# dfki-asr/morphablegraphs

Hardware: AMD Instinct MI355X
Metric: motion-primitive samples scored+back-projected/sec; fraction of HBM roofline (higher is better)
Workload: dtype f32; 1 GPU; walk primitive L=40 F=156 D=79 NB=31 GMM k=8, batch=8192 candidates/GPU (BASELINE.json configs[1]); candidates_per_gpu=8192, global_candidates=8192, collective=none, clock_ramp_steps=1500

## Files before the change

include/mg_hip.h:

```cpp
#ifndef MG_HIP_H
#define MG_HIP_H

#include <stdint.h>

#ifdef __cplusplus
extern "C" {
#endif

typedef struct mg_context mg_context;
typedef struct mg_primitive mg_primitive;
typedef struct mg_time_grid mg_time_grid;
typedef struct mg_constraint_set mg_constraint_set;

enum {
    MG_OK = 0,
    MG_ERR_INVALID_ARGUMENT = -1,
    MG_ERR_NO_DEVICE = -2,
    MG_ERR_HIP = -3,
    MG_ERR_UNSUPPORTED = -4,
    MG_ERR_NOT_POSITIVE_DEFINITE = -5,
    MG_ERR_OUT_OF_MEMORY = -6
};

enum { MG_F32 = 0, MG_F64 = 1 };

enum {
    MG_PATH_AUTO = 0,
    MG_PATH_MFMA = 1,
    MG_PATH_DIRECT = 2
};

typedef struct mg_primitive_desc {
    int32_t n_basis;
    int32_t n_dim;
    int32_t n_components;
    int32_t n_canonical_frames;
    int32_t n_gmm;
    int32_t eigen_is_transposed;
    const double *eigen_vectors;
    const double *mean_vector;
    const double *translation_maxima;
    const double *knots;
    const double *gmm_weights;
    const double *gmm_means;
    const double *gmm_covars;
    int32_t n_gmm_dims;
    int32_t n_time_components;
    int32_t n_basis_time;
    int32_t reserved;
    const double *eigen_vectors_time;
    const double *mean_time_vector;
    const double *knots_time;
} mg_primitive_desc;

enum { MG_CONSTRAINT_POSITION = 0, MG_CONSTRAINT_DIRECTION_2D = 1, MG_CONSTRAINT_JOINT_POSITION = 2,
       MG_CONSTRAINT_JOINT_MIDPOINT = 3, MG_CONSTRAINT_JOINT_ORIENTATION = 4, MG_CONSTRAINT_LOOK_AT = 5,
       MG_CONSTRAINT_POSE = 6 ,
       MG_CONSTRAINT_VALUE_POSITION = 7, MG_CONSTRAINT_VALUE_HEADING = 8 };
#define MG_MAX_CHAIN 32
typedef struct mg_keyframe_constraint {
    int32_t type;
    int32_t joint;
    double canonical_keyframe;
    double weight_factor;
    double target[3];
    double ref_dir[3];
    int32_t joint2;
    int32_t reserved;
} mg_keyframe_constraint;

typedef struct mg_pose_constraint {
    int32_t n_points;
    int32_t has_velocity;
    const int32_t *joints;
    const double *points;
    const double *weights;
    double velocity[3];
} mg_pose_constraint;
#define MG_MAX_POSE_POINTS 64

typedef struct mg_skeleton_desc {
    int32_t n_joints;
    int32_t reserved;
    const int32_t *parents;
    const double *offsets;
    const int32_t *quat_channel;
} mg_skeleton_desc;

#define MG_ALIGN_START_POSE (-1)
typedef struct mg_alignment_desc {
    int32_t joint;
    int32_t reserved;
    double position[3];
    double heading[2];
    double ref_dir[3];
} mg_alignment_desc;

const char *mg_version(void);
const char *mg_last_error(void);
const char *mg_status_string(int status);

int mg_context_create(int device, void *stream, mg_context **out);
void mg_context_destroy(mg_context *ctx);
int mg_context_set_stream(mg_context *ctx, void *stream);
int mg_context_set_reserved_cus(mg_context *ctx, int32_t n);
#define MG_OPT_FORCE_VALU_SCORE 0
#define MG_OPT_FORCE_VALU_SAMPLE 1
#define MG_OPT_RING_SLOTS 2
#define MG_OPT_CHUNK_WINDOW 3
#define MG_OPT_CHUNK_SAMPLES 4
#define MG_OPT_FRAMES_KERNEL 5
#define MG_OPT_PLACED_FAST_PCT 6
#define MG_OPT_OPTIONS_STEP 7
#define MG_OPT_PLAIN_MALLOC 8
#define MG_OPT_GMM_KERNEL 9
#define MG_OPT_SCORE_KERNEL 10
#define MG_OPT_ROOT_MODE 11
#define MG_OPT_PLACED_HOLD 12
#define MG_OPT_TRAJECTORY_LANES 13
#define MG_OPT_TRAJECTORY_SEARCH 14
#define MG_OPT_COUNT 15
int mg_context_set_option(mg_context *ctx, int32_t option, int32_t value);
int mg_context_arena_begin(mg_context *ctx, int64_t block_bytes);
int mg_context_arena_end(mg_context *ctx);
int mg_context_arena_bytes(mg_context *ctx, int64_t *reserved, int64_t *used);
int mg_context_synchronize(mg_context *ctx);
int mg_context_device_info(mg_context *ctx, char *name, int32_t *n_cu, int64_t *total_mem);

int mg_device_malloc(mg_context *ctx, int64_t bytes, void **out_dev);
int mg_device_free(mg_context *ctx, void *ptr_dev);
int mg_context_trim_outputs(mg_context *ctx);
int mg_context_output_bytes(mg_context *ctx, int64_t *reserved, int64_t *in_use, int32_t *n_regions, int32_t *n_fast);
int mg_device_malloc_chunked(mg_context *ctx, int64_t bytes, int64_t chunk_bytes, void **out_dev);
int mg_device_malloc_placed(mg_context *ctx, int64_t bytes, int32_t max_candidates, void **out_dev, double *info4);
int mg_device_probe_placement(mg_context *ctx, void *buf_dev, int64_t bytes, double *info4);
int mg_device_placement_info(mg_context *ctx, const void *buf_dev, double *info4, double *tbps);
int mg_memcpy_h2d(mg_context *ctx, void *dst_dev, const void *src, int64_t bytes);
int mg_memcpy_d2h(mg_context *ctx, void *dst, const void *src_dev, int64_t bytes);
int mg_memset(mg_context *ctx, void *dst_dev, int value, int64_t bytes);

int mg_profile_enable(mg_context *ctx, int enabled);
int mg_profile_reset(mg_context *ctx);
int mg_profile_get(mg_context *ctx, int slot, double *total_ms, int64_t *launches);
int mg_profile_get_samples(mg_context *ctx, int slot, float *out_ms, int64_t capacity, int64_t *n);

#define MG_DIST_ID_BYTES 128
int mg_dist_unique_id(void *id_out);
int mg_dist_init(mg_context *ctx, int32_t rank, int32_t n_ranks, const void *id);
int mg_dist_all_gather(mg_context *ctx, const void *local_dev, void *gathered_dev, int64_t count, int dtype);
int mg_dist_broadcast(mg_context *ctx, void *buf_dev, int64_t bytes, int32_t root);
int mg_dist_finalize(mg_context *ctx);
int mg_dist_preflight(mg_context *ctx);
int mg_dist_info(mg_context *ctx, int32_t *out3);

int mg_primitive_create(mg_context *ctx, const mg_primitive_desc *desc, mg_primitive **out);
void mg_primitive_destroy(mg_primitive *prim);
int mg_primitive_info(const mg_primitive *prim, int32_t *out8);
int mg_primitive_info2(const mg_primitive *prim, int32_t *out4);
int mg_primitive_root_mode(const mg_primitive *prim, int32_t *split, double *estimate);
int mg_primitive_get_precisions_cholesky(const mg_primitive *prim, double *out);

int mg_time_function_canonical(mg_primitive *prim, const void *gamma_dev, int gamma_dtype, int64_t n_samples, int64_t ld,
                               double *out_dev);
int mg_time_function_canonical_host(mg_primitive *prim, const void *gamma, int gamma_dtype, int64_t n_samples, int64_t ld,
                                    double *out);
int mg_time_function_sample(mg_primitive *prim, const void *gamma, int dtype, int64_t n, int64_t ld, double speed, double *times, int32_t *lengths,
                            int32_t t_cap, double *canonical_out);
int mg_time_function_sample_rows(mg_primitive *prim, const void *gamma, int dtype, int64_t n, int64_t ld, double speed, double *times, int32_t *lengths,
                                 int32_t t_cap, int64_t row_pitch, double *canonical_out);
int mg_back_project_frames_at(mg_primitive *prim, const void *latents, int dtype, int64_t n, int64_t ld, const double *times, const int32_t *lengths,
                              int32_t t_cap, void *out, int out_dtype);

int mg_time_grid_create(mg_primitive *prim, const double *times, int32_t n_times, mg_time_grid **out);
void mg_time_grid_destroy(mg_time_grid *grid);
mg_time_grid *mg_primitive_canonical_grid(mg_primitive *prim);
int mg_time_grid_size(const mg_time_grid *grid);
int mg_time_grid_get_tables(const mg_time_grid *grid, int32_t *i0, double *weights, double *times);

int mg_joint_positions(mg_context *ctx, const mg_skeleton_desc *skeleton, const int32_t *joints, int32_t n_out,
                       const double *frames_dev, int64_t n_frames, int32_t n_dim, double *out_dev);

typedef struct mg_trajectory mg_trajectory;
int mg_trajectory_create(mg_primitive *prim, const double *control_points, int32_t n_points, int32_t granularity, mg_trajectory **out);
void mg_trajectory_destroy(mg_trajectory *trajectory);
int mg_score_trajectory(mg_primitive *prim, const mg_trajectory *trajectory, const mg_time_grid *grid, const void *latents_dev,
                        int latent_dtype, int64_t n_samples, int64_t ld, double min_u, double weight, const mg_alignment_desc *alignment,
                        double *errors_dev, int accumulate, double *residuals_dev);
int mg_score_trajectories(int32_t n, mg_primitive *const *prims, const mg_trajectory *const *trajectories, const void *const *latents_dev,
                          int latent_dtype, int64_t n_samples, const int64_t *ld, const double *min_u, const double *weight,
                          const mg_alignment_desc *const *alignments, double *const *errors_dev, int accumulate);

int mg_score_trajectory_points(mg_primitive *prim, const mg_trajectory *trajectory, const double *points_dev, int64_t n_samples, int32_t n_times,
                               double min_u, double weight, double *errors_dev, int accumulate, double *residuals_dev);

int mg_trajectory_closest_points(mg_primitive *prim, const mg_trajectory *trajectory, const double *points_dev, int64_t n_samples, int32_t n_times,
                                 double min_u, double *params_dev, double *distances_dev, int32_t *evaluations_dev);

#define MG_FRAME_CA_POSITION 1
#define MG_FRAME_DISCRETE_TRAJECTORY 2
#define MG_FRAME_LOCAL_TRAJECTORY 3
#define MG_FRAME_TRAJECTORY_SET 4
#define MG_FRAME_JOINT_ROTATION 5
#define MG_FRAME_JOINT_TRAJECTORY 6
#define MG_FRAME_MAX_JOINTS 8
typedef struct mg_frame_constraint_desc {
    int32_t type;
    int32_t n_frames;
    int32_t n_points;
    int32_t n_joints;
    double weight;
    double target[3];
    int32_t axis_on[3];
    int32_t quat_channel;
    const double *points_dev;
    double start_arc;
    const mg_trajectory *trajectories[MG_FRAME_MAX_JOINTS];
    double arc0[MG_FRAME_MAX_JOINTS], range_start[MG_FRAME_MAX_JOINTS], range_end[MG_FRAME_MAX_JOINTS];
    int32_t has_range[MG_FRAME_MAX_JOINTS];
    double quaternion[4];
} mg_frame_constraint_desc;
int mg_align_frames(mg_primitive *prim, double *frames_dev, int64_t n_samples, int32_t n_times, const double *vals_dev, int32_t n_vals,
                    const mg_alignment_desc *alignment);
int mg_frame_constraint_width(const mg_frame_constraint_desc *constraint, int32_t n_times);
int mg_score_frame_constraint(mg_primitive *prim, const mg_frame_constraint_desc *constraint, const double *tracks_dev, int64_t n_samples,
                              int32_t n_times, int32_t n_joints, double *errors_dev, int accumulate, double *residuals_dev);
typedef struct mg_track_plan mg_track_plan;
int mg_track_plan_create(mg_primitive *prim, const mg_skeleton_desc *skeleton, int32_t n_requests, const int32_t *n_joints, const int32_t *joints,
                         int32_t align_joint, mg_track_plan **out);
void mg_track_plan_destroy(mg_track_plan *plan);
int mg_joint_tracks(mg_track_plan *plan, const void *latents, int dtype, int64_t n_samples, int64_t ld, const mg_alignment_desc *alignment,
                    const mg_time_grid *const *grids, double *const *tracks_dev);
int mg_score_frame_constraints(mg_primitive *prim, int32_t n_constraints, const mg_frame_constraint_desc *const *constraints, const double *const *tracks_dev,
                               const int32_t *n_times, const int32_t *n_joints, int64_t n_samples, double *errors_dev, int accumulate,
                               double *const *residuals_dev);

#define MG_TRACK_MAX_REQUESTS 4
#define MG_FRAME_LIST_MAX 4
int mg_options_frame_lists(int32_t n_options, mg_primitive *const *prims, mg_track_plan *const *plans, const void *const *latents_dev, int latent_dtype,
                           int64_t n_samples, const int64_t *ld, const mg_alignment_desc *const *alignments, const mg_time_grid *const *grids,
                           double *const *tracks_dev, const int32_t *n_constraints, const mg_frame_constraint_desc *const *constraints,
                           const int32_t *request_of, double *const *errors_dev, void *results_dev, int64_t result_stride, void *results_host);


int mg_back_project_frames(mg_primitive *prim, const mg_time_grid *grid,
                           const void *latents_dev, int latent_dtype, int64_t n_samples, int64_t ld,
                           float *frames_dev, int path);

int mg_back_project_frames_f64(mg_primitive *prim, const mg_time_grid *grid,
                               const void *latents_dev, int latent_dtype, int64_t n_samples, int64_t ld,
                               double *frames_dev);

int mg_back_project_coeffs(mg_primitive *prim, const void *latents_dev, int latent_dtype,
                           int64_t n_samples, int64_t ld, void *coeffs_dev, int out_dtype);

int mg_spline_evaluate(mg_primitive *prim, const mg_time_grid *grid, const double *coeffs_dev,
                       int64_t n_splines, double *frames_dev);

int mg_gmm_log_prob(mg_primitive *prim, const void *x_dev, int x_dtype, int64_t n_samples, int64_t ld,
                    void *logp_dev, int out_dtype);

int mg_gmm_log_prob_jac(mg_primitive *prim, const void *x_dev, int x_dtype, int64_t n_samples, int64_t ld,
                        double *jac_dev);

int mg_gmm_sample(mg_primitive *prim, int64_t n_samples, const int64_t *counts, uint64_t seed,
                  void *x_dev, int x_dtype, int64_t ld, int32_t *component_dev);
int mg_gmm_sample_rows(mg_primitive *prim, int64_t n_samples, const int64_t *counts, uint64_t seed, int64_t row_begin, int64_t row_count,
                       void *x_dev, int x_dtype, int64_t ld, int32_t *component_dev);

int mg_constraint_set_create(mg_primitive *prim, const mg_keyframe_constraint *cons, int32_t n,
                             mg_constraint_set **out);
int mg_constraint_set_create_fk(mg_primitive *prim, const mg_skeleton_desc *skeleton,
                                const mg_keyframe_constraint *cons, int32_t n, mg_constraint_set **out);
int mg_constraint_set_create_aligned(mg_primitive *prim, const mg_skeleton_desc *skeleton,
                                     const mg_keyframe_constraint *cons, int32_t n,
// ... 166 lines not shown
```

morphablegraphs_amd/_capi.py:

```python
import ctypes as C
import functools
import itertools
import os

import numpy as np

HERE = os.path.dirname(os.path.abspath(__file__))
LIB_PATH = os.path.join(HERE, "csrc", "libmg_hip.so")

MG_OK = 0
MG_ERR_INVALID_ARGUMENT = -1
MG_ERR_UNSUPPORTED = -4
MG_F32, MG_F64 = 0, 1
MG_PATH_AUTO, MG_PATH_MFMA, MG_PATH_DIRECT = 0, 1, 2
MG_ALIGN_START_POSE = -1
MG_OPT_FORCE_VALU_SCORE, MG_OPT_FORCE_VALU_SAMPLE, MG_OPT_RING_SLOTS, MG_OPT_CHUNK_WINDOW, MG_OPT_CHUNK_SAMPLES = 0, 1, 2, 3, 4
MG_OPT_FRAMES_KERNEL = 5
MG_OPT_PLACED_FAST_PCT = 6
MG_OPT_OPTIONS_STEP = 7
MG_OPT_PLAIN_MALLOC = 8
MG_OPT_GMM_KERNEL = 9
MG_OPT_SCORE_KERNEL = 10
MG_OPT_ROOT_MODE = 11
MG_OPT_PLACED_HOLD = 12
MG_OPT_TRAJECTORY_LANES = 13
MG_OPT_TRAJECTORY_SEARCH = 14
MG_OPT_COUNT = 15
MG_CONSTRAINT_POSITION, MG_CONSTRAINT_DIRECTION_2D, MG_CONSTRAINT_JOINT_POSITION = 0, 1, 2
MG_CONSTRAINT_JOINT_MIDPOINT, MG_CONSTRAINT_JOINT_ORIENTATION, MG_CONSTRAINT_LOOK_AT, MG_CONSTRAINT_POSE = 3, 4, 5, 6
MG_CONSTRAINT_VALUE_POSITION, MG_CONSTRAINT_VALUE_HEADING = 7, 8
PROFILE_SLOTS = {"frames": 0, "gmm_log_prob": 1, "score_constraints": 2, "argmin": 3,
                 "gmm_sample": 4, "spline_evaluate": 5, "step": 6, "options_step": 7, "joint_tracks": 8, "frame_constraints": 9, "trajectory": 10,
                 "cluster_tree_search": 11, "walk_frames": 12}
MG_TREE_MAX_DEPTH, MG_TREE_MAX_CHILDREN, MG_TREE_MAX_CANDIDATES = 64, 256, 64
MG_TREE_TIE, MG_TREE_NO_RESULT, MG_TREE_OVERFLOW, MG_TREE_NO_MEAN = 1, 2, 4, 8
MG_KD_MAX_DEPTH = 64
TREE_SEARCH_RECORD = np.dtype([("row", "<i8"), ("leaf", "<i4"), ("flags", "<i4"), ("evaluations", "<i8"), ("value", "<f8")])
MG_WALK_MAX_STEPS = 64
MG_WALK_TILE = 32
MG_FUSED_MAX_OPTIONS = 24


@functools.lru_cache(maxsize=None)
def _option_record(stride):
    return np.dtype([("index", "<i8"), ("error", "<f8"), ("latent", "<f8", ((stride - 16) // 8,))])


def option_records(raw, m, stride):
    return raw[:m * stride].copy().view(_option_record(stride))


EXPORTED_SYMBOLS = [
    "mg_version", "mg_last_error", "mg_status_string",
    "mg_context_create", "mg_context_destroy", "mg_context_set_stream", "mg_context_set_reserved_cus", "mg_context_set_option", "mg_context_arena_begin", "mg_context_arena_end", "mg_context_arena_bytes", "mg_context_synchronize",
    "mg_dist_unique_id", "mg_dist_init", "mg_dist_all_gather", "mg_dist_finalize", "mg_dist_preflight", "mg_dist_info",
    "mg_context_device_info", "mg_device_malloc", "mg_device_malloc_chunked", "mg_device_malloc_placed", "mg_device_probe_placement", "mg_device_placement_info", "mg_device_free", "mg_context_trim_outputs", "mg_context_output_bytes", "mg_memcpy_h2d", "mg_memcpy_d2h",
    "mg_memset", "mg_profile_enable", "mg_profile_reset", "mg_profile_get", "mg_profile_get_samples",
    "mg_primitive_create", "mg_primitive_destroy", "mg_primitive_info", "mg_primitive_info2", "mg_primitive_root_mode", "mg_primitive_get_precisions_cholesky",
    "mg_time_function_canonical", "mg_time_function_canonical_host", "mg_time_function_sample", "mg_time_function_sample_rows", "mg_back_project_frames_at",
    "mg_trajectory_create", "mg_trajectory_destroy", "mg_score_trajectory", "mg_score_trajectories", "mg_score_trajectory_points", "mg_trajectory_closest_points", "mg_joint_positions",
    "mg_time_grid_create", "mg_time_grid_destroy", "mg_primitive_canonical_grid", "mg_time_grid_size",
    "mg_time_grid_get_tables",
    "mg_back_project_frames", "mg_back_project_frames_f64", "mg_back_project_coeffs", "mg_spline_evaluate",
    "mg_gmm_log_prob", "mg_gmm_sample", "mg_constraint_set_create", "mg_constraint_set_destroy",
    "mg_score_constraints", "mg_argmin_first", "mg_argmin_first_dev", "mg_step_frames_and_logp", "mg_step_plan", "mg_step_plan_for", "mg_step_plan_dtype",
    "mg_back_project_frames_host", "mg_back_project_frames_f64_host", "mg_back_project_coeffs_host",
    "mg_spline_evaluate_host", "mg_gmm_log_prob_host", "mg_gmm_sample_host", "mg_score_constraints_host",
    "mg_score_constraint_residuals", "mg_objective_error_and_naturalness", "mg_gmm_log_prob_jac", "mg_score_constraint_residuals_host",
    "mg_gmm_log_prob_jac_host", "mg_constraint_set_create_fk", "mg_constraint_set_create_aligned", "mg_constraint_set_create_full", "mg_constraint_set_update", "mg_best_candidate", "mg_best_candidate_host",
    "mg_align_frames", "mg_frame_constraint_width", "mg_score_frame_constraint", "mg_score_frame_constraints", "mg_options_frame_lists", "mg_track_plan_create", "mg_track_plan_destroy", "mg_joint_tracks",
    "mg_score_constraint_residuals_chained", "mg_option_step", "mg_options_step", "mg_options_step_device_counts", "mg_option_step_rows", "mg_options_step_rows", "mg_gmm_sample_rows", "mg_dist_broadcast",
    "mg_cluster_tree_create", "mg_cluster_tree_destroy", "mg_cluster_tree_search", "mg_cluster_tree_search_host",
    "mg_cluster_tree_create_kd", "mg_kmeans_segments", "mg_gmm_em_fit",
    "mg_spline_fit_batch", "mg_pca_fit", "mg_pca_project", "mg_pca_backproject",
    "mg_dtw_distance_grids", "mg_dtw_paths", "mg_warp_motions", "mg_dtw_pair_costs",
    "mg_keyframe_distances", "mg_segment_search",
    "mg_align_motions_spatially", "mg_prepare_aligned_frames",
    "mg_walk_frames", "mg_walk_frames_host",
]


class MGError(RuntimeError):
    def __init__(self, status, message):
        RuntimeError.__init__(self, "libmg_hip status %d: %s" % (status, message))
        self.status = status


class PrimitiveDesc(C.Structure):
    _fields_ = [("n_basis", C.c_int32), ("n_dim", C.c_int32), ("n_components", C.c_int32),
                ("n_canonical_frames", C.c_int32), ("n_gmm", C.c_int32), ("eigen_is_transposed", C.c_int32),
                ("eigen_vectors", C.c_void_p), ("mean_vector", C.c_void_p), ("translation_maxima", C.c_void_p),
                ("knots", C.c_void_p), ("gmm_weights", C.c_void_p), ("gmm_means", C.c_void_p),
                ("gmm_covars", C.c_void_p), ("n_gmm_dims", C.c_int32), ("n_time_components", C.c_int32),
                ("n_basis_time", C.c_int32), ("reserved", C.c_int32), ("eigen_vectors_time", C.c_void_p),
                ("mean_time_vector", C.c_void_p), ("knots_time", C.c_void_p)]


class KeyframeConstraint(C.Structure):
    _fields_ = [("type", C.c_int32), ("joint", C.c_int32), ("canonical_keyframe", C.c_double),
                ("weight_factor", C.c_double), ("target", C.c_double * 3), ("ref_dir", C.c_double * 3),
                ("joint2", C.c_int32), ("reserved", C.c_int32)]


class PoseConstraintDesc(C.Structure):
    _fields_ = [("n_points", C.c_int32), ("has_velocity", C.c_int32), ("joints", C.c_void_p), ("points", C.c_void_p),
                ("weights", C.c_void_p), ("velocity", C.c_double * 3)]


class SkeletonDesc(C.Structure):
    _fields_ = [("n_joints", C.c_int32), ("reserved", C.c_int32), ("parents", C.c_void_p), ("offsets", C.c_void_p),
                ("quat_channel", C.c_void_p)]


class AlignmentDesc(C.Structure):
    _fields_ = [("joint", C.c_int32), ("reserved", C.c_int32), ("position", C.c_double * 3), ("heading", C.c_double * 2),
                ("ref_dir", C.c_double * 3)]


MG_FRAME_CA_POSITION, MG_FRAME_DISCRETE_TRAJECTORY, MG_FRAME_LOCAL_TRAJECTORY, MG_FRAME_TRAJECTORY_SET, MG_FRAME_JOINT_ROTATION = 1, 2, 3, 4, 5
MG_FRAME_JOINT_TRAJECTORY = 6
MG_FRAME_MAX_JOINTS = 8
MG_TRACK_MAX_REQUESTS = 4
MG_FRAME_LIST_MAX = 4


class FrameConstraintDesc(C.Structure):
    _fields_ = [("type", C.c_int32), ("n_frames", C.c_int32), ("n_points", C.c_int32), ("n_joints", C.c_int32), ("weight", C.c_double),
                ("target", C.c_double * 3), ("axis_on", C.c_int32 * 3), ("quat_channel", C.c_int32), ("points_dev", C.c_void_p),
                ("start_arc", C.c_double), ("trajectories", C.c_void_p * MG_FRAME_MAX_JOINTS), ("arc0", C.c_double * MG_FRAME_MAX_JOINTS),
                ("range_start", C.c_double * MG_FRAME_MAX_JOINTS), ("range_end", C.c_double * MG_FRAME_MAX_JOINTS),
                ("has_range", C.c_int32 * MG_FRAME_MAX_JOINTS), ("quaternion", C.c_double * 4)]


def _quat_mul(a, b):
    return np.array([a[0] * b[0] - a[1] * b[1] - a[2] * b[2] - a[3] * b[3], a[0] * b[1] + a[1] * b[0] + a[2] * b[3] - a[3] * b[2],
                     a[0] * b[2] - a[1] * b[3] + a[2] * b[0] + a[3] * b[1], a[0] * b[3] + a[1] * b[2] - a[2] * b[1] + a[3] * b[0]])


def rotate_by_quaternion(q, v):
    q = np.asarray(q, dtype=np.float64)
    q = q / np.linalg.norm(q)
    v = np.asarray(v, dtype=np.float64)
    u = q[1:]
    return v + 2.0 * (q[0] * np.cross(u, v) + np.cross(u, np.cross(u, v)))


class Skeleton(object):

    _serials = itertools.count(1)

    def __init__(self, joints, animated_joints):
        self.serial = next(Skeleton._serials)
        self.names = [j[0] for j in joints]
        index = {n: i for i, n in enumerate(self.names)}
        if len(index) != len(self.names):
            raise ValueError("duplicate joint names")
        self.parents = np.array([-1 if j[1] is None else index[j[1]] for j in joints], dtype=np.int32)
        self.offsets = np.ascontiguousarray([j[2] for j in joints], dtype=np.float64).reshape(len(joints), 3)
        self.animated_joints = list(animated_joints)
        chan = {n: 3 + 4 * i for i, n in enumerate(self.animated_joints)}
        self.quat_channel = np.array([chan.get(n, -1) for n in self.names], dtype=np.int32)
        if self.parents[0] != -1 or np.any(self.parents[1:] >= np.arange(1, len(joints))) or np.any(self.parents[1:] < 0):
            raise ValueError("joint 0 must be the root and parents must precede their children")

    def index(self, joint):
        return int(joint) if isinstance(joint, (int, np.integer)) else self.names.index(joint)

    def indices(self, joints):
        return np.ascontiguousarray([self.index(j) for j in joints], dtype=np.int32)

    def chain(self, joint):
        out, j = [], self.index(joint)
        while j >= 0:
            out.insert(0, j)
            j = int(self.parents[j])
        return out

    def heading(self, frame, joint=0, ref_dir=(0.0, 0.0, 1.0)):
        frame = np.asarray(frame, dtype=np.float64)
        q = np.array([1.0, 0.0, 0.0, 0.0])
# ... 1289 lines not shown
```

morphablegraphs_amd/csrc/mg_options.hip:

```cpp
#include <algorithm>
#include <cstring>

#include <hip/hip_ext.h>

#include "mg_internal.h"
#include "mg_gmm_device.h"
#include "mg_score_device.h"

#define MG_FUSED_MAX_OPTIONS 24
#define MG_FUSED_WAVES_PER_SIMD 3

struct mg_fused_static {
    const double *cpack;
    const double *meanpad;
    const double *Wpack;
    const double *bpad;
    mg_score_args sa;
    void *x;
    void *result;
    void *result_host;
    double cumw[MG_SAMPLE_ARG_K];
    int32_t K, Lg, KKg, KK, JT, RT;
};

struct mg_fused_dyn {
    uint64_t seed[MG_FUSED_MAX_OPTIONS];
    int32_t counts[MG_FUSED_MAX_OPTIONS][MG_SAMPLE_ARG_K];
    int32_t wg0[MG_FUSED_MAX_OPTIONS + 1];
    int32_t tile0[MG_FUSED_MAX_OPTIONS], tile_end[MG_FUSED_MAX_OPTIONS];
    int64_t row_lo, row_hi;
    unsigned long long *flags_host;
    unsigned long long seq;
    int32_t fenced;
};

struct mg_fused_devcounts {
    int32_t counts[MG_FUSED_MAX_OPTIONS][MG_SAMPLE_ARG_K];
    int32_t tile_end[MG_FUSED_MAX_OPTIONS];
};

struct mg_fused_partial { double v; int64_t i; double row[4 * MG_MAX_KK]; };

#define MG_COUNTS_TAG 0x636e7473u
struct mg_counts_args {
    uint64_t seed[MG_FUSED_MAX_OPTIONS];
    int64_t n;
};
__device__ __forceinline__ void mg_counts_draw(const mg_fused_static &o, const uint64_t seed, const int64_t n, mg_fused_devcounts *__restrict__ dc, const int k,
                                               int (*below)[MG_SAMPLE_ARG_K]) {
    const int tid = threadIdx.x, lane = tid & 63, wave = tid >> 6;
    const int K = o.K;
    double cum[MG_SAMPLE_ARG_K];
#pragma unroll
    for (int c = 0; c < MG_SAMPLE_ARG_K; c++) cum[c] = o.cumw[c];
#pragma unroll
    for (int c = 0; c < MG_SAMPLE_ARG_K; c++) cum[c] = c < K - 1 ? cum[c] : -1.0;
    int lt[MG_SAMPLE_ARG_K];
#pragma unroll
    for (int c = 0; c < MG_SAMPLE_ARG_K; c++) lt[c] = 0;
    const int64_t groups = (n + 3) >> 2;
    for (int64_t j = tid; j < groups; j += 256) {
        uint32_t rr[4];
        mg_philox4x32_10((uint32_t)j, (uint32_t)(j >> 32), 0u, MG_COUNTS_TAG, (uint32_t)seed, (uint32_t)(seed >> 32), rr);
#pragma unroll
        for (int e = 0; e < 4; e++) {
            const double u = 4 * j + e < n ? ((double)rr[e] + 0.5) * (1.0 / 4294967296.0) : 2.0;
#pragma unroll
            for (int c = 0; c < MG_SAMPLE_ARG_K; c++) lt[c] += u < cum[c] ? 1 : 0;
        }
    }
#pragma unroll
    for (int c = 0; c < MG_SAMPLE_ARG_K; c++) {
        int v = lt[c];
        for (int off = 32; off > 0; off >>= 1) v += __shfl_down(v, off, 64);
        if (lane == 0) below[wave][c] = v;
    }
    __syncthreads();
    if (tid < MG_SAMPLE_ARG_K) {
        const int c = tid;
        auto cum_at = [&](int q) { return q < 0 ? 0 : (q < K - 1 ? below[0][q] + below[1][q] + below[2][q] + below[3][q] : (int)n); };
        const int cnt = c < K ? cum_at(c) - cum_at(c - 1) : 0;
        dc->counts[k][c] = cnt;
        int tiles = (cnt + 15) / 16;
        for (int off = 8; off > 0; off >>= 1) tiles += __shfl_down(tiles, off, 16);
        if (c == 0) dc->tile_end[k] = tiles;
    }
    __syncthreads();
}
__global__ __launch_bounds__(256) void mg_options_counts_kernel(const mg_fused_static *__restrict__ tab, const mg_counts_args a,
                                                               mg_fused_devcounts *__restrict__ dc) {
    __shared__ int below[4][MG_SAMPLE_ARG_K];
    mg_counts_draw(tab[blockIdx.x], a.seed[blockIdx.x], a.n, dc, blockIdx.x, below);
}

template <bool X_F64, bool DYN_DEV>
__global__ __launch_bounds__(256, MG_FUSED_WAVES_PER_SIMD) void mg_options_fused_kernel(const mg_fused_static *__restrict__ tab, const mg_fused_dyn dyn_arg,
                                                              const mg_fused_devcounts *__restrict__ dyn_dev,
                                                              mg_fused_devcounts *__restrict__ next_dev, int32_t *__restrict__ counts_host,
                                                              const int n_options, const int wave_doubles,
                                                              mg_fused_partial *__restrict__ partials, int32_t *__restrict__ counters) {
    const mg_fused_dyn &dyn = dyn_arg;
    extern __shared__ __attribute__((aligned(16))) unsigned char smem[];
    __shared__ double sv[4];
    __shared__ int64_t si[4];
    __shared__ int s_last;
    __shared__ int s_below[4][MG_SAMPLE_ARG_K];
    const int tid = threadIdx.x, lane = tid & 63;
    const int wave = __builtin_amdgcn_readfirstlane(tid >> 6);
    const int cl = lane & 15, g = lane >> 4;
    const int wg = blockIdx.x;
    int k = 0;
    while (k + 1 < n_options && wg >= dyn.wg0[k + 1]) k++;
    const mg_fused_static &o = tab[k];
    const int K = o.K, Lg = o.Lg, KKg = o.KKg, KK = o.KK, JT = o.JT, RT = o.RT, L = o.sa.L, n = o.sa.n;
    const int64_t ld = o.sa.ld;
    const int ZS = 4 * KKg + 1, vs = RT * 16 + 1;
    double *zt = (double *)smem + (size_t)wave * wave_doubles;
    double *vals = zt + 16 * ZS;
    double *resid = vals + 16 * vs;

    const int64_t t = dyn.tile0[k] + (int64_t)(wg - dyn.wg0[k]) * 4 + wave;
    const int64_t row_lo = dyn.row_lo, row_hi = dyn.row_hi;
    int c = 0;
    int64_t row_c = 0, tile_c = 0, rows_next, tiles_next;
    int32_t cnts[MG_SAMPLE_ARG_K];
#pragma unroll
    for (int q = 0; q < MG_SAMPLE_ARG_K; q++) cnts[q] = DYN_DEV ? dyn_dev->counts[k][q] : dyn.counts[k][q];
    const int tile_end_k = DYN_DEV ? dyn_dev->tile_end[k] : dyn.tile_end[k];
    if (DYN_DEV && counts_host && wg == dyn.wg0[k] && tid < MG_SAMPLE_ARG_K) {
        int mine = cnts[0];
#pragma unroll
        for (int q = 1; q < MG_SAMPLE_ARG_K; q++) mine = tid == q ? cnts[q] : mine;
        __hip_atomic_store(counts_host + k * MG_SAMPLE_ARG_K + tid, mine, __ATOMIC_RELAXED, __HIP_MEMORY_SCOPE_SYSTEM);
    }
    for (;;) {
        int cnt = cnts[0];
#pragma unroll
        for (int q = 1; q < MG_SAMPLE_ARG_K; q++) cnt = c == q ? cnts[q] : cnt;
        rows_next = row_c + cnt;
        tiles_next = tile_c + (cnt + 15) / 16;
        if (c + 1 < K && t >= tiles_next) { c++; row_c = rows_next; tile_c = tiles_next; }
        else break;
    }
    const bool active = t < tiles_next && t < tile_end_k;
    double best = INFINITY;
    int64_t bi = INT64_MAX;
    if (active) {
        const int64_t row0 = row_c + (t - tile_c) * 16;
        const int nrow = (int)((rows_next - row0) < 16 ? (rows_next - row0) : 16);
        const uint64_t seed = dyn.seed[k];
        for (int e = lane; e < 16 * KKg; e += 64) {
            const int r = e & 15, q = e >> 4;
            const int64_t b = row0 + r;
            double z4[4];
            mg_normal4(b, q, seed, z4);
#pragma unroll
            for (int j = 0; j < 4; j++) zt[r * ZS + 4 * q + j] = z4[j];
        }
        asm volatile("s_waitcnt lgkmcnt(0)" ::: "memory");
        double za[MG_MAX_KK];
#pragma unroll
        for (int kk = 0; kk < MG_MAX_KK; kk++) za[kk] = (kk < KKg && 4 * kk + g < Lg) ? zt[cl * ZS + 4 * kk + g] : 0.0;
#pragma unroll
        for (int it = 0; it < MG_MAX_KK / 4; it++) {
            if (it < JT) {
                const double m = o.meanpad[((size_t)c * JT + it) * 16 + cl];
                mg_f64x4 acc = {m, m, m, m};
                typedef double mg_f64x2 __attribute__((ext_vector_type(2)));
                const mg_f64x2 *cp2 = (const mg_f64x2 *)(o.cpack + (size_t)K * JT * KKg * 64) + (((size_t)c * JT + it) * (KKg / 2)) * 64 + lane;
#pragma unroll
                for (int q = 0; q < MG_MAX_KK / 2; q++)
                    if (2 * q < KKg && 2 * q < 4 * (it + 1)) {
                        const mg_f64x2 v = cp2[q * 64];
                        acc = __builtin_amdgcn_mfma_f64_16x16x4f64(za[2 * q], v[0], acc, 0, 0, 0);
                        acc = __builtin_amdgcn_mfma_f64_16x16x4f64(za[2 * q + 1], v[1], acc, 0, 0, 0);
                    }
                const int i = 16 * it + cl;
#pragma unroll
                for (int r = 0; r < 4; r++) {
                    const int row = g + 4 * r;
                    if (i < Lg) {
                        const double xv = X_F64 ? acc[r] : (double)(float)acc[r];
                        zt[row * ZS + i] = xv;
                        const int64_t gr = row0 + row;
                        if (row < nrow && gr >= row_lo && gr < row_hi) {
                            if (X_F64) ((double *)o.x)[(gr - row_lo) * ld + i] = acc[r];
                            else ((float *)o.x)[(gr - row_lo) * ld + i] = (float)acc[r];
                        }
                    }
                }
            }
        }
        asm volatile("s_waitcnt lgkmcnt(0)" ::: "memory");
        double xf[MG_MAX_KK];
#pragma unroll
        for (int kk = 0; kk < MG_MAX_KK; kk++) xf[kk] = (kk < KK && 4 * kk + g < L && cl < nrow) ? zt[cl * ZS + 4 * kk + g] : 0.0;
        for (int rt = 0; rt < RT; rt++) {
            const double *wp = o.Wpack + ((size_t)rt * KK) * 64 + lane;
            const double c0 = o.bpad[rt * 16 + cl];
            mg_f64x4 acc = {c0, c0, c0, c0};
#pragma unroll
            for (int kk = 0; kk < MG_MAX_KK; kk++)
                if (kk < KK) acc = __builtin_amdgcn_mfma_f64_16x16x4f64(xf[kk], wp[kk * 64], acc, 0, 0, 0);
#pragma unroll
            for (int r = 0; r < 4; r++) vals[(g + 4 * r) * vs + rt * 16 + cl] = acc[r];
        }
        asm volatile("s_waitcnt lgkmcnt(0)" ::: "memory");
        for (int e = lane; e < 16 * n; e += 64) {
            const int cand = e & 15, cc = e >> 4;
            const double *v = vals + cand * vs;
            resid[cc * 16 + cand] = mg_constraint_residual(o.sa, cc, [&](int row) { return v[row]; });
        }
        asm volatile("s_waitcnt lgkmcnt(0)" ::: "memory");
        if (lane < nrow && row0 + lane >= row_lo && row0 + lane < row_hi) {
            double err = 0.0;
            for (int cc = 0; cc < n; cc++) err += resid[cc * 16 + lane];
            ((double *)o.sa.out)[row0 + lane - row_lo] = err;
            if (err < INFINITY) { best = err; bi = row0 + lane; }
        }
    }
    for (int off = 32; off > 0; off >>= 1) {
        const double ov = __shfl_down(best, off, 64);
        const long long oi = __shfl_down((long long)bi, off, 64);
        mg_min_combine(best, bi, ov, (int64_t)oi);
    }
    if (lane == 0) { sv[wave] = best; si[wave] = bi; }
    __syncthreads();
    const int nwg = dyn.wg0[k + 1] - dyn.wg0[k];
    best = sv[0]; bi = si[0];
    for (int w = 1; w < 4; w++) mg_min_combine(best, bi, sv[w], si[w]);
    {
        const int64_t pub = bi != INT64_MAX ? bi : row_lo;
        const int64_t row0 = row_c + (t - tile_c) * 16;
        const int64_t row_end = rows_next < row0 + 16 ? rows_next : row0 + 16;
        if (active && pub >= row0 && pub < row_end && lane < Lg)
            __hip_atomic_store(&partials[wg].row[lane], zt[(int)(pub - row0) * ZS + lane], __ATOMIC_RELAXED, __HIP_MEMORY_SCOPE_AGENT);
    }
    if (tid == 0) {
        __hip_atomic_store(&partials[wg].v, best, __ATOMIC_RELAXED, __HIP_MEMORY_SCOPE_AGENT);
        __hip_atomic_store(&partials[wg].i, bi, __ATOMIC_RELAXED, __HIP_MEMORY_SCOPE_AGENT);
    }
    asm volatile("s_waitcnt vmcnt(0)" ::: "memory");
    if (dyn.fenced) __builtin_amdgcn_fence(__ATOMIC_RELEASE, "agent");
    __syncthreads();
    if (tid == 0) {
        const int old = __hip_atomic_fetch_add(&counters[k], 1, __ATOMIC_RELAXED, __HIP_MEMORY_SCOPE_AGENT);
        s_last = (old == nwg - 1) ? 1 : 0;
    }
    __syncthreads();
    if (dyn.fenced) __builtin_amdgcn_fence(__ATOMIC_ACQUIRE, "agent");
    if (DYN_DEV && next_dev != nullptr && wg == dyn.wg0[k]) {
        mg_counts_draw(o, dyn.seed[k] + 1, o.sa.B, next_dev, k, s_below);
    }
    if (!s_last) return;
    best = INFINITY; bi = INT64_MAX;
    for (int w = tid; w < nwg; w += 256) {
        const mg_fused_partial *pp = &partials[dyn.wg0[k] + w];
        const double pv = __hip_atomic_load(&pp->v, __ATOMIC_RELAXED, __HIP_MEMORY_SCOPE_AGENT);
        const int64_t pi = __hip_atomic_load(&pp->i, __ATOMIC_RELAXED, __HIP_MEMORY_SCOPE_AGENT);
        mg_min_combine(best, bi, pv, pi);
    }
    for (int off = 32; off > 0; off >>= 1) {
        const double ov = __shfl_down(best, off, 64);
        const long long oi = __shfl_down((long long)bi, off, 64);
        mg_min_combine(best, bi, ov, (int64_t)oi);
    }
    if (lane == 0) { sv[wave] = best; si[wave] = bi; }
    __syncthreads();
    if (tid == 0) {
        for (int w = 1; w < 4; w++) mg_min_combine(best, bi, sv[w], si[w]);
        si[1] = bi;
        if (bi == INT64_MAX || bi < row_lo || bi >= row_hi) { bi = row_lo; best = INFINITY; }
        ((int64_t *)o.result)[0] = bi;
        ((double *)o.result)[1] = best;
        if (o.result_host) {
            __hip_atomic_store((int64_t *)o.result_host, bi, __ATOMIC_RELAXED, __HIP_MEMORY_SCOPE_SYSTEM);
            __hip_atomic_store((double *)o.result_host + 1, best, __ATOMIC_RELAXED, __HIP_MEMORY_SCOPE_SYSTEM);
        }
        si[0] = bi;
        counters[k] = 0;
    }
    __syncthreads();
    const int64_t widx = si[1];
    if (tid == 0) s_last = 0;
    __syncthreads();
    if (widx != INT64_MAX)
        for (int w = tid; w < nwg; w += 256)
            if (__hip_atomic_load(&partials[dyn.wg0[k] + w].i, __ATOMIC_RELAXED, __HIP_MEMORY_SCOPE_AGENT) == widx) s_last = w;
    __syncthreads();
    const mg_fused_partial *win = &partials[dyn.wg0[k] + s_last];
    double *row = (double *)((char *)o.result + 16);
    double *row_h = o.result_host ? (double *)((char *)o.result_host + 16) : nullptr;
    for (int i = tid; i < Lg; i += 256) {
        const double v = __hip_atomic_load(&win->row[i], __ATOMIC_RELAXED, __HIP_MEMORY_SCOPE_AGENT);
        row[i] = v;
        if (row_h) __hip_atomic_store(row_h + i, v, __ATOMIC_RELAXED, __HIP_MEMORY_SCOPE_SYSTEM);
    }
    if (dyn.flags_host) {
        asm volatile("s_waitcnt vmcnt(0)" ::: "memory");
        if (dyn.fenced) __builtin_amdgcn_fence(__ATOMIC_RELEASE, "");
        __syncthreads();
        if (tid == 0) __hip_atomic_store(dyn.flags_host + k, dyn.seq, __ATOMIC_RELAXED, __HIP_MEMORY_SCOPE_SYSTEM);
    }
}

int mg_options_fused_attributes() {
    MG_HIP_CHECK(hipFuncSetAttribute((const void *)mg_options_fused_kernel<true, false>, hipFuncAttributeMaxDynamicSharedMemorySize, 160 * 1024 - 1024));
    MG_HIP_CHECK(hipFuncSetAttribute((const void *)mg_options_fused_kernel<false, false>, hipFuncAttributeMaxDynamicSharedMemorySize, 160 * 1024 - 1024));
    MG_HIP_CHECK(hipFuncSetAttribute((const void *)mg_options_fused_kernel<true, true>, hipFuncAttributeMaxDynamicSharedMemorySize, 160 * 1024 - 1024));
    MG_HIP_CHECK(hipFuncSetAttribute((const void *)mg_options_fused_kernel<false, true>, hipFuncAttributeMaxDynamicSharedMemorySize, 160 * 1024 - 1024));
    return MG_OK;
}

bool mg_options_can_fuse(int32_t n_options, mg_primitive *const *prims, const mg_constraint_set *const *csets, int64_t n) {
    if (n_options < 1 || n_options > MG_FUSED_MAX_OPTIONS || n < 1 || n > (int64_t)1 << 30) return false;
    mg_context *ctx = prims[0]->ctx;
    if (ctx->opt[MG_OPT_FORCE_VALU_SAMPLE] || ctx->opt[MG_OPT_FORCE_VALU_SCORE] || ctx->opt[MG_OPT_OPTIONS_STEP] == 1) return false;
    for (int k = 0; k < n_options; k++) {
        const mg_primitive *p = prims[k];
        const mg_constraint_set *cs = csets[k];
        if (!mg_gmm_sample_takes_host_prefix(p) || p->KK <= 0 || !cs || cs->prim != p || !cs->d_Wpack) return false;
        const int64_t wd = 16 * (4 * p->KKg + 1) + 16 * (cs->RT * 16 + 1) + 16 * (int64_t)std::max(cs->n, 1);
        if (4 * wd * 8 > 150 * 1024) return false;
    }
    return true;
}

int mg_launch_options_fused(int32_t n_options, mg_primitive *const *prims, const mg_constraint_set *const *csets, int64_t n,
                            const int64_t *const *counts, const uint64_t *seeds, void *const *x_dev, int xdt, const int64_t *ld,
                            double *const *errors_dev, void *results_dev, int64_t result_stride, int64_t row_begin, int64_t row_count,
                            void *records_host, int32_t *counts_host, unsigned long long *flags_host, unsigned long long seq) {
    mg_context *ctx = prims[0]->ctx;
    const bool dev_counts = counts == nullptr;
    if (dev_counts && (row_begin != 0 || row_count != n)) {
        mg_set_error("mg_options_step_device_counts: the device draws the counts of whole draws only");
        return MG_ERR_UNSUPPORTED;
    }
    mg_counts_args ca;
    memset(&ca, 0, sizeof(ca));
    ca.n = n;
    std::vector<mg_fused_static> tab((size_t)n_options);
    mg_fused_dyn dyn;
    memset(&dyn, 0, sizeof(dyn));
    memset(tab.data(), 0, tab.size() * sizeof(mg_fused_static));
    int wave_doubles = 0;
    for (int k = 0; k < n_options; k++) {
        mg_primitive *p = prims[k];
        const mg_constraint_set *cs = csets[k];
        mg_fused_static &o = tab[k];
        o.cpack = p->d_gcholpack; o.meanpad = p->d_gmeanpad; o.Wpack = cs->d_Wpack; o.bpad = cs->d_bpad;
        mg_score_args &a = o.sa;
        a = mg_score_args_of(cs, p->L);
        a.lat = x_dev[k]; a.out = errors_dev[k]; a.B = n; a.ld = ld[k];
        o.x = x_dev[k]; o.result = (char *)results_dev + (size_t)k * result_stride;
        o.result_host = records_host ? (char *)records_host + (size_t)k * result_stride : nullptr;
        {
            double wsum = 0.0, acc = 0.0;
            for (int c = 0; c < p->K; c++) wsum += p->gw[c];
            for (int c = 0; c < p->K && c < MG_SAMPLE_ARG_K; c++) { acc += p->gw[c]; o.cumw[c] = acc / wsum; }
        }
        o.K = p->K; o.Lg = p->Lg; o.KKg = p->KKg; o.KK = p->KK; o.JT = (p->Lg + 15) / 16; o.RT = cs->RT;
        wave_doubles = std::max(wave_doubles, 16 * (4 * p->KKg + 1) + 16 * (cs->RT * 16 + 1) + 16 * std::max(cs->n, 1));
        int64_t tiles = 0, rows = 0, t_first = -1, t_last = -1;
        if (dev_counts) {
            ca.seed[k] = seeds[k];
            dyn.seed[k] = seeds[k];
            dyn.tile0[k] = 0;
            dyn.wg0[k + 1] = dyn.wg0[k] + (int32_t)((n / 16 + p->K + 3) / 4);
            continue;
        }
        for (int c = 0; c < p->K; c++) {
            if (counts[k][c] < 0 || counts[k][c] > n) { mg_set_error("mg_options_step: counts[%d][%d] out of range", k, c); return MG_ERR_INVALID_ARGUMENT; }
            dyn.counts[k][c] = (int32_t)counts[k][c];
            if (t_first < 0 && row_begin < rows + counts[k][c]) t_first = tiles + (row_begin - rows) / 16;
            if (t_last < 0 && row_begin + row_count - 1 < rows + counts[k][c]) t_last = tiles + (row_begin + row_count - 1 - rows) / 16;
            rows += counts[k][c];
            tiles += (counts[k][c] + 15) / 16;
        }
        if (rows != n) { mg_set_error("mg_options_step: counts of option %d sum to %lld, expected %lld", k, (long long)rows, (long long)n); return MG_ERR_INVALID_ARGUMENT; }
        dyn.seed[k] = seeds[k];
        dyn.tile0[k] = (int32_t)t_first;
        dyn.tile_end[k] = (int32_t)(t_last + 1);
        dyn.wg0[k + 1] = dyn.wg0[k] + (int32_t)((t_last + 1 - t_first + 3) / 4);
    }
    dyn.row_lo = row_begin; dyn.row_hi = row_begin + row_count;
    dyn.flags_host = flags_host; dyn.seq = seq;
    dyn.fenced = ctx->opt[MG_OPT_OPTIONS_STEP] == 3 ? 1 : 0;
    const int total_wg = dyn.wg0[n_options];
    const size_t tab_bytes = tab.size() * sizeof(mg_fused_static);
    if (!ctx->fused_tab_dev || ctx->fused_tab_host.size() != tab_bytes || memcmp(ctx->fused_tab_host.data(), tab.data(), tab_bytes) != 0) {
        MG_HIP_CHECK(hipStreamSynchronize(ctx->stream));
        if (!ctx->fused_tab_dev) MG_HIP_CHECK(hipMalloc(&ctx->fused_tab_dev, MG_FUSED_MAX_OPTIONS * sizeof(mg_fused_static)));
        MG_HIP_CHECK(hipMemcpy(ctx->fused_tab_dev, tab.data(), tab_bytes, hipMemcpyHostToDevice));
        ctx->fused_tab_host.assign((const unsigned char *)tab.data(), (const unsigned char *)tab.data() + tab_bytes);
    }
    if (!ctx->fused_counters) {
        MG_HIP_CHECK(hipMalloc(&ctx->fused_counters, MG_FUSED_MAX_OPTIONS * sizeof(int32_t)));
        MG_HIP_CHECK(hipMemset(ctx->fused_counters, 0, MG_FUSED_MAX_OPTIONS * sizeof(int32_t)));
    }
    if (ctx->fused_partials_n < total_wg) {
        MG_HIP_CHECK(hipStreamSynchronize(ctx->stream));
        if (ctx->fused_partials) MG_HIP_CHECK(hipFree(ctx->fused_partials));
        ctx->fused_partials = nullptr; ctx->fused_partials_n = 0;
        const int cap = std::max(total_wg, 2048);
        MG_HIP_CHECK(hipMalloc(&ctx->fused_partials, (size_t)cap * sizeof(mg_fused_partial)));
        ctx->fused_partials_n = cap;
    }
    const size_t lds = (size_t)4 * wave_doubles * 8;
    hipEvent_t ev0 = nullptr, ev1 = nullptr;
    const bool timed = mg_prof_kernel(ctx, 7, -1, &ev0, &ev1);
    const mg_fused_static *tabd = (const mg_fused_static *)ctx->fused_tab_dev;
    mg_fused_partial *part = (mg_fused_partial *)ctx->fused_partials;
    int32_t *ctr = (int32_t *)ctx->fused_counters;
    if (dev_counts) {
        if (!ctx->fused_dyn_dev) MG_HIP_CHECK(hipMalloc(&ctx->fused_dyn_dev, 2 * sizeof(mg_fused_devcounts)));
        auto &fn = ctx->fused_next;
        bool hit = fn.valid && fn.n_options == n_options && fn.n == n && ctx->opt[MG_OPT_OPTIONS_STEP] != 2;
        for (int k = 0; k < n_options && hit; k++) hit = fn.seeds[k] == seeds[k] && fn.prims[k] == (const void *)prims[k];
        const int slot = hit ? fn.slot : 0;
        mg_fused_devcounts *dd = (mg_fused_devcounts *)ctx->fused_dyn_dev + slot, *dnext = (mg_fused_devcounts *)ctx->fused_dyn_dev + (slot ^ 1);
        if (!hit) hipLaunchKernelGGL(mg_options_counts_kernel, dim3(n_options), dim3(256), 0, ctx->stream, tabd, ca, dd);
        fn.valid = false; fn.n_options = n_options; fn.n = n; fn.slot = slot ^ 1;
        for (int k = 0; k < n_options; k++) { fn.seeds[k] = seeds[k] + 1; fn.prims[k] = (const void *)prims[k]; }
        if (xdt == MG_F64)
            hipExtLaunchKernelGGL((mg_options_fused_kernel<true, true>), dim3(total_wg), dim3(256), lds, ctx->stream, timed ? ev0 : nullptr, timed ? ev1 : nullptr, 0,
                                  tabd, dyn, (const mg_fused_devcounts *)dd, dnext, counts_host, (int)n_options, wave_doubles, part, ctr);
        else
            hipExtLaunchKernelGGL((mg_options_fused_kernel<false, true>), dim3(total_wg), dim3(256), lds, ctx->stream, timed ? ev0 : nullptr, timed ? ev1 : nullptr, 0,
                                  tabd, dyn, (const mg_fused_devcounts *)dd, dnext, counts_host, (int)n_options, wave_doubles, part, ctr);
    } else if (xdt == MG_F64) {
        hipExtLaunchKernelGGL((mg_options_fused_kernel<true, false>), dim3(total_wg), dim3(256), lds, ctx->stream, timed ? ev0 : nullptr, timed ? ev1 : nullptr, 0,
                              tabd, dyn, (const mg_fused_devcounts *)nullptr, (mg_fused_devcounts *)nullptr, (int32_t *)nullptr, (int)n_options, wave_doubles, part, ctr);
    } else {
        hipExtLaunchKernelGGL((mg_options_fused_kernel<false, false>), dim3(total_wg), dim3(256), lds, ctx->stream, timed ? ev0 : nullptr, timed ? ev1 : nullptr, 0,
                              tabd, dyn, (const mg_fused_devcounts *)nullptr, (mg_fused_devcounts *)nullptr, (int32_t *)nullptr, (int)n_options, wave_doubles, part, ctr);
    }
    MG_HIP_CHECK(hipGetLastError());
    if (dev_counts) ctx->fused_next.valid = true;
    return MG_OK;
}
```

Before: 106.3 million samples/s.

## Cap fused options grid and let each wave process a run of tiles

The fused options kernel now bounds its grid to about waves-per-SIMD times CU count (overridable through a new MG_OPT_OPTIONS_GRID option) and gives each wave a contiguous run of T tiles instead of exactly one. The per-tile argmin is reduced within the wave every iteration, and the winning latent row is stashed in LDS so it can be published at the end. The aim is to cut workgroup launch and cross-workgroup partial-reduction overhead and to make the grid fit resident occupancy. The costs are a serialised loop per wave, extra per-tile reductions and readfirstlane work, and 4 KB more static LDS, with less dynamic LDS left as a result.

```diff
diff --git a/include/mg_hip.h b/include/mg_hip.h
--- a/include/mg_hip.h
+++ b/include/mg_hip.h
@@ -119,7 +119,8 @@
 #define MG_OPT_PLACED_HOLD 12
 #define MG_OPT_TRAJECTORY_LANES 13
 #define MG_OPT_TRAJECTORY_SEARCH 14
-#define MG_OPT_COUNT 15
+#define MG_OPT_OPTIONS_GRID 15
+#define MG_OPT_COUNT 16
 int mg_context_set_option(mg_context *ctx, int32_t option, int32_t value);
 int mg_context_arena_begin(mg_context *ctx, int64_t block_bytes);
 int mg_context_arena_end(mg_context *ctx);
diff --git a/morphablegraphs_amd/_capi.py b/morphablegraphs_amd/_capi.py
--- a/morphablegraphs_amd/_capi.py
+++ b/morphablegraphs_amd/_capi.py
@@ -25,7 +25,8 @@
 MG_OPT_PLACED_HOLD = 12
 MG_OPT_TRAJECTORY_LANES = 13
 MG_OPT_TRAJECTORY_SEARCH = 14
-MG_OPT_COUNT = 15
+MG_OPT_OPTIONS_GRID = 15
+MG_OPT_COUNT = 16
 MG_CONSTRAINT_POSITION, MG_CONSTRAINT_DIRECTION_2D, MG_CONSTRAINT_JOINT_POSITION = 0, 1, 2
 MG_CONSTRAINT_JOINT_MIDPOINT, MG_CONSTRAINT_JOINT_ORIENTATION, MG_CONSTRAINT_LOOK_AT, MG_CONSTRAINT_POSE = 3, 4, 5, 6
 MG_CONSTRAINT_VALUE_POSITION, MG_CONSTRAINT_VALUE_HEADING = 7, 8
diff --git a/morphablegraphs_amd/csrc/mg_options.hip b/morphablegraphs_amd/csrc/mg_options.hip
--- a/morphablegraphs_amd/csrc/mg_options.hip
+++ b/morphablegraphs_amd/csrc/mg_options.hip
@@ -27,6 +27,7 @@
     uint64_t seed[MG_FUSED_MAX_OPTIONS];
     int32_t counts[MG_FUSED_MAX_OPTIONS][MG_SAMPLE_ARG_K];
     int32_t wg0[MG_FUSED_MAX_OPTIONS + 1];
+    int32_t run[MG_FUSED_MAX_OPTIONS];
     int32_t tile0[MG_FUSED_MAX_OPTIONS], tile_end[MG_FUSED_MAX_OPTIONS];
     int64_t row_lo, row_hi;
     unsigned long long *flags_host;
@@ -91,6 +92,14 @@
                                                                mg_fused_devcounts *__restrict__ dc) {
     __shared__ int below[4][MG_SAMPLE_ARG_K];
     mg_counts_draw(tab[blockIdx.x], a.seed[blockIdx.x], a.n, dc, blockIdx.x, below);
+}
+
+__device__ __forceinline__ double mg_first_lane(double v) {
+    return __hiloint2double(__builtin_amdgcn_readfirstlane(__double2hiint(v)), __builtin_amdgcn_readfirstlane(__double2loint(v)));
+}
+__device__ __forceinline__ int64_t mg_first_lane(int64_t v) {
+    const uint32_t lo = (uint32_t)__builtin_amdgcn_readfirstlane((int)(uint32_t)v), hi = (uint32_t)__builtin_amdgcn_readfirstlane((int)(uint32_t)((uint64_t)v >> 32));
+    return (int64_t)(((uint64_t)hi << 32) | lo);
 }
 
 template <bool X_F64, bool DYN_DEV>
@@ -105,9 +114,9 @@
     __shared__ int64_t si[4];
     __shared__ int s_last;
     __shared__ int s_below[4][MG_SAMPLE_ARG_K];
+    __shared__ double s_row[4][4 * MG_MAX_KK];
     const int tid = threadIdx.x, lane = tid & 63;
     const int wave = __builtin_amdgcn_readfirstlane(tid >> 6);
-    const int cl = lane & 15, g = lane >> 4;
     const int wg = blockIdx.x;
     int k = 0;
     while (k + 1 < n_options && wg >= dyn.wg0[k + 1]) k++;
@@ -119,36 +128,50 @@
     double *vals = zt + 16 * ZS;
     double *resid = vals + 16 * vs;
 
-    const int64_t t = dyn.tile0[k] + (int64_t)(wg - dyn.wg0[k]) * 4 + wave;
+    const int T = dyn.run[k];
+    const int t_begin = dyn.tile0[k] + ((wg - dyn.wg0[k]) * 4 + wave) * T;
     const int64_t row_lo = dyn.row_lo, row_hi = dyn.row_hi;
     int c = 0;
-    int64_t row_c = 0, tile_c = 0, rows_next, tiles_next;
+    int row_c = 0, tile_c = 0, rows_next, tiles_next;
     int32_t cnts[MG_SAMPLE_ARG_K];
 #pragma unroll
     for (int q = 0; q < MG_SAMPLE_ARG_K; q++) cnts[q] = DYN_DEV ? dyn_dev->counts[k][q] : dyn.counts[k][q];
-    const int tile_end_k = DYN_DEV ? dyn_dev->tile_end[k] : dyn.tile_end[k];
+    const int tile_end_k = __builtin_amdgcn_readfirstlane(DYN_DEV ? dyn_dev->tile_end[k] : dyn.tile_end[k]);
     if (DYN_DEV && counts_host && wg == dyn.wg0[k] && tid < MG_SAMPLE_ARG_K) {
         int mine = cnts[0];
 #pragma unroll
         for (int q = 1; q < MG_SAMPLE_ARG_K; q++) mine = tid == q ? cnts[q] : mine;
         __hip_atomic_store(counts_host + k * MG_SAMPLE_ARG_K + tid, mine, __ATOMIC_RELAXED, __HIP_MEMORY_SCOPE_SYSTEM);
     }
+    const int t_stop = t_begin + T < tile_end_k ? t_begin + T : tile_end_k;
     for (;;) {
         int cnt = cnts[0];
 #pragma unroll
         for (int q = 1; q < MG_SAMPLE_ARG_K; q++) cnt = c == q ? cnts[q] : cnt;
         rows_next = row_c + cnt;
         tiles_next = tile_c + (cnt + 15) / 16;
-        if (c + 1 < K && t >= tiles_next) { c++; row_c = rows_next; tile_c = tiles_next; }
+        if (c + 1 < K && t_begin >= tiles_next) { c++; row_c = rows_next; tile_c = tiles_next; }
         else break;
     }
-    const bool active = t < tiles_next && t < tile_end_k;
+    c = __builtin_amdgcn_readfirstlane(c); row_c = __builtin_amdgcn_readfirstlane(row_c); tile_c = __builtin_amdgcn_readfirstlane(tile_c);
+    rows_next = __builtin_amdgcn_readfirstlane(rows_next); tiles_next = __builtin_amdgcn_readfirstlane(tiles_next);
+    const uint64_t seed = dyn.seed[k];
     double best = INFINITY;
     int64_t bi = INT64_MAX;
-    if (active) {
+    bool have_lo = false;
+    for (int t = t_begin; t < t_stop; t++) {
+        while (c + 1 < K && t >= tiles_next) {
+            c++; row_c = rows_next; tile_c = tiles_next;
+            const int cnt = __builtin_amdgcn_readfirstlane(DYN_DEV ? dyn_dev->counts[k][c] : dyn.counts[k][c]);
+            rows_next = row_c + cnt;
+            tiles_next = tile_c + (cnt + 15) / 16;
+        }
+        if (t >= tiles_next) break;
+        int lane_t = tid & 63;
+        asm volatile("" : "+v"(lane_t));
+        const int lane = lane_t, cl = lane & 15, g = lane >> 4;
         const int64_t row0 = row_c + (t - tile_c) * 16;
         const int nrow = (int)((rows_next - row0) < 16 ? (rows_next - row0) : 16);
-        const uint64_t seed = dyn.seed[k];
         for (int e = lane; e < 16 * KKg; e += 64) {
             const int r = e & 15, q = e >> 4;
             const int64_t b = row0 + r;
@@ -212,30 +235,40 @@
             resid[cc * 16 + cand] = mg_constraint_residual(o.sa, cc, [&](int row) { return v[row]; });
         }
         asm volatile("s_waitcnt lgkmcnt(0)" ::: "memory");
+        double tv = INFINITY;
+        int64_t ti = INT64_MAX;
         if (lane < nrow && row0 + lane >= row_lo && row0 + lane < row_hi) {
             double err = 0.0;
             for (int cc = 0; cc < n; cc++) err += resid[cc * 16 + lane];
             ((double *)o.sa.out)[row0 + lane - row_lo] = err;
-            if (err < INFINITY) { best = err; bi = row0 + lane; }
-        }
-    }
-    for (int off = 32; off > 0; off >>= 1) {
-        const double ov = __shfl_down(best, off, 64);
-        const long long oi = __shfl_down((long long)bi, off, 64);
-        mg_min_combine(best, bi, ov, (int64_t)oi);
+            if (err < INFINITY) { tv = err; ti = row0 + lane; }
+        }
+        for (int off = 8; off > 0; off >>= 1) {
+            const double ov = __shfl_down(tv, off, 64);
+            const long long oi = __shfl_down((long long)ti, off, 64);
+            mg_min_combine(tv, ti, ov, (int64_t)oi);
+        }
+        tv = mg_first_lane(tv); ti = mg_first_lane(ti);
+        mg_min_combine(best, bi, tv, ti);
+        best = mg_first_lane(best); bi = mg_first_lane(bi);
+        const bool lead = ti != INT64_MAX && bi == ti;
+        const int64_t row_end = rows_next < row0 + 16 ? rows_next : row0 + 16;
+        const bool holds_lo = bi == INT64_MAX && row_lo >= row0 && row_lo < row_end;
+        if (lead || holds_lo) {
+            const int64_t pub = lead ? bi : row_lo;
+            if (lane < Lg) s_row[wave][lane] = zt[(int)(pub - row0) * ZS + lane];
+            have_lo = !lead;
+        }
+        asm volatile("s_waitcnt lgkmcnt(0)" ::: "memory");
     }
     if (lane == 0) { sv[wave] = best; si[wave] = bi; }
     __syncthreads();
     const int nwg = dyn.wg0[k + 1] - dyn.wg0[k];
+    const int64_t mine = bi;
     best = sv[0]; bi = si[0];
     for (int w = 1; w < 4; w++) mg_min_combine(best, bi, sv[w], si[w]);
-    {
-        const int64_t pub = bi != INT64_MAX ? bi : row_lo;
-        const int64_t row0 = row_c + (t - tile_c) * 16;
-        const int64_t row_end = rows_next < row0 + 16 ? rows_next : row0 + 16;
-        if (active && pub >= row0 && pub < row_end && lane < Lg)
-            __hip_atomic_store(&partials[wg].row[lane], zt[(int)(pub - row0) * ZS + lane], __ATOMIC_RELAXED, __HIP_MEMORY_SCOPE_AGENT);
-    }
+    if ((bi != INT64_MAX ? mine == bi : have_lo) && lane < Lg)
+        __hip_atomic_store(&partials[wg].row[lane], s_row[wave][lane], __ATOMIC_RELAXED, __HIP_MEMORY_SCOPE_AGENT);
     if (tid == 0) {
         __hip_atomic_store(&partials[wg].v, best, __ATOMIC_RELAXED, __HIP_MEMORY_SCOPE_AGENT);
         __hip_atomic_store(&partials[wg].i, bi, __ATOMIC_RELAXED, __HIP_MEMORY_SCOPE_AGENT);
@@ -304,11 +337,12 @@
     }
 }
 
+#define MG_FUSED_DYN_LDS (160 * 1024 - 4096)
 int mg_options_fused_attributes() {
-    MG_HIP_CHECK(hipFuncSetAttribute((const void *)mg_options_fused_kernel<true, false>, hipFuncAttributeMaxDynamicSharedMemorySize, 160 * 1024 - 1024));
-    MG_HIP_CHECK(hipFuncSetAttribute((const void *)mg_options_fused_kernel<false, false>, hipFuncAttributeMaxDynamicSharedMemorySize, 160 * 1024 - 1024));
-    MG_HIP_CHECK(hipFuncSetAttribute((const void *)mg_options_fused_kernel<true, true>, hipFuncAttributeMaxDynamicSharedMemorySize, 160 * 1024 - 1024));
-    MG_HIP_CHECK(hipFuncSetAttribute((const void *)mg_options_fused_kernel<false, true>, hipFuncAttributeMaxDynamicSharedMemorySize, 160 * 1024 - 1024));
+    MG_HIP_CHECK(hipFuncSetAttribute((const void *)mg_options_fused_kernel<true, false>, hipFuncAttributeMaxDynamicSharedMemorySize, MG_FUSED_DYN_LDS));
+    MG_HIP_CHECK(hipFuncSetAttribute((const void *)mg_options_fused_kernel<false, false>, hipFuncAttributeMaxDynamicSharedMemorySize, MG_FUSED_DYN_LDS));
+    MG_HIP_CHECK(hipFuncSetAttribute((const void *)mg_options_fused_kernel<true, true>, hipFuncAttributeMaxDynamicSharedMemorySize, MG_FUSED_DYN_LDS));
+    MG_HIP_CHECK(hipFuncSetAttribute((const void *)mg_options_fused_kernel<false, true>, hipFuncAttributeMaxDynamicSharedMemorySize, MG_FUSED_DYN_LDS));
     return MG_OK;
 }
 
@@ -344,6 +378,7 @@
     memset(&dyn, 0, sizeof(dyn));
     memset(tab.data(), 0, tab.size() * sizeof(mg_fused_static));
     int wave_doubles = 0;
+    int64_t slots[MG_FUSED_MAX_OPTIONS];
     for (int k = 0; k < n_options; k++) {
         mg_primitive *p = prims[k];
         const mg_constraint_set *cs = csets[k];
@@ -366,7 +401,7 @@
             ca.seed[k] = seeds[k];
             dyn.seed[k] = seeds[k];
             dyn.tile0[k] = 0;
-            dyn.wg0[k + 1] = dyn.wg0[k] + (int32_t)((n / 16 + p->K + 3) / 4);
+            slots[k] = n / 16 + p->K;
             continue;
         }
         for (int c = 0; c < p->K; c++) {
@@ -381,7 +416,22 @@
         dyn.seed[k] = seeds[k];
         dyn.tile0[k] = (int32_t)t_first;
         dyn.tile_end[k] = (int32_t)(t_last + 1);
-        dyn.wg0[k + 1] = dyn.wg0[k] + (int32_t)((t_last + 1 - t_first + 3) / 4);
+        slots[k] = t_last + 1 - t_first;
+    }
+    {
+        int64_t total_slots = 0, wg_one_tile = 0;
+        for (int k = 0; k < n_options; k++) { total_slots += slots[k]; wg_one_tile += (slots[k] + 3) / 4; }
+        int64_t cap = (int64_t)MG_FUSED_WAVES_PER_SIMD * std::max(1, ctx->n_cu);
+        if (ctx->opt[MG_OPT_OPTIONS_GRID] > 0) cap = ctx->opt[MG_OPT_OPTIONS_GRID];
+        cap = std::max<int64_t>(cap, n_options);
+        for (int k = 0; k < n_options; k++) {
+            int64_t w = (slots[k] + 3) / 4;
+            if (wg_one_tile > cap) w = std::min(w, 1 + (cap - n_options) * slots[k] / total_slots);
+            const int64_t T = (slots[k] + 4 * w - 1) / (4 * w);
+            w = (slots[k] + 4 * T - 1) / (4 * T);
+            dyn.run[k] = (int32_t)T;
+            dyn.wg0[k + 1] = dyn.wg0[k] + (int32_t)w;
+        }
     }
     dyn.row_lo = row_begin; dyn.row_hi = row_begin + row_count;
     dyn.flags_host = flags_host; dyn.seq = seq;
```

Measured after the change: 106.2 million samples/s, median of 2. About the same (-0.1%).
